# wafgo/rt-depth-map

Measured on AMD Instinct MI355X. Metric: stereo-pairs/sec, 1280x720 d=64 9x9 SAD, higher is better.
Workload: dtype u8

## Files before the change

rt-depth-map_amd/csrc/k_search_ring.hip:

```cpp
#include "rtdm_select.h"
#include "rtdm_border.h"
#include "rtdm_border2.h"

#include <cmath>
#include <cstdlib>
#include <type_traits>
#include <utility>

#ifndef RING_ABL
#define RING_ABL 0
#endif
#ifndef RING_LDS_SELECT
#define RING_LDS_SELECT 1
#endif
#ifndef RING_MINREC
#define RING_MINREC 1
#endif
#ifndef RING_W3_LIMIT
#define RING_W3_LIMIT 112
#endif
#ifndef RING_STATIC_SLOTS
#define RING_STATIC_SLOTS 1
#endif
#ifndef RING_DIRECT_LOADS
#define RING_DIRECT_LOADS 1
#endif
#ifndef RING_B64REC
#define RING_B64REC 1
#endif
#ifndef RING_MINREC96
#define RING_MINREC96 1
#endif
#ifndef RING_SPLIT_SELECT
#define RING_SPLIT_SELECT 0
#endif

#ifdef RING_STAMPS
__device__ unsigned long long ring_stamps[8];
#define RING_STAMP(i) do { unsigned long long t_; asm volatile("s_memtime %0\n\ts_waitcnt lgkmcnt(0)" : "=s"(t_) :: "memory"); \
                           stamp_sum[i] += t_ - stamp_last; stamp_last = t_; } while (0)
extern "C" void rtdm_debug_ring_stamps(unsigned long long* out, int reset)
{
    (void)hipMemcpyFromSymbol(out, HIP_SYMBOL(ring_stamps), sizeof(unsigned long long) * 8);
    if (reset) { unsigned long long z[8] = {0}; (void)hipMemcpyToSymbol(HIP_SYMBOL(ring_stamps), z, sizeof z); }
}
#else
#define RING_STAMP(i) do { } while (0)
#endif

namespace rtdm {

struct RingGeom {
    int x0, nx;
    int rs;
    uint32_t lastmask;
    int tiles, strips;
    unsigned nitems;
    unsigned chunk;
    uint32_t rdelta;
    int rebase;
    unsigned nborder;
    int bgx, bgy;
    int b2;
};

#ifndef RING_RPG96
#define RING_RPG96 4
#endif
#ifndef RING_RPG128
#define RING_RPG128 4
#endif
#ifndef RING_RPG256
#define RING_RPG256 4
#endif
__host__ __device__ constexpr int ring_rpg(int D, int LPP)
{ return D == 256 ? RING_RPG256 : D >= 192 ? 4 : D == 128 ? RING_RPG128 : D == 96 ? RING_RPG96 : LPP; }

template <int D, int WS, int LPP = 2>
struct RingCfg {
    static constexpr int RPG = ring_rpg(D, LPP);
    static constexpr bool SPLIT = LPP != 2 || D >= 48 || (D == 32 && (WS == 9 || WS == 5)) || (RING_SPLIT_SELECT && RING_LDS_SELECT);
    static constexpr bool MINREC = SPLIT && RING_MINREC && !(D == 128 && RPG == 8) && !(D == 96 && !RING_MINREC96);
    static_assert(RPG == LPP || MINREC, "GroupSelect's lane reductions need one owner per lane of a pixel");
    static constexpr bool B64 = MINREC && D == 64 && RING_B64REC;
    using Rec = SelRecord<D, MINREC || !SPLIT, B64>;
    static constexpr int NP = (WS + 3) / 4;
    static constexpr int W1 = WS + 1;
    static constexpr int PPW = 64 / LPP;
    static constexpr int DL = D / LPP;
    static constexpr int NGL = DL / 4;
    static constexpr int NRL = DL / 2;
    static constexpr int NW = NGL + NP - 1;
    static constexpr int LWD = PPW + NP;
    static constexpr int RWD = PPW + D / 4 + NP;
    static constexpr int ITEMS = (LWD + RWD + 63) / 64;
    static constexpr int SLOT = ITEMS * 64;
    static constexpr int TRIP = (W1 % RPG == 0) ? W1 : (2 * W1 % RPG == 0) ? 2 * W1 : 4 * W1;
    static_assert(W1 % 2 == 0 && TRIP % RPG == 0 && TRIP % W1 == 0, "block sizes are odd");
    static constexpr bool STATIC_SLOTS = RING_STATIC_SLOTS && ITEMS == 1 && TRIP % 4 == 0;
    static constexpr int NSLOT = STATIC_SLOTS ? 4 : 3;
    static constexpr int STG = (NSLOT * SLOT + (W1 + RPG) * PPW / 2 + 3) & ~3;
    static constexpr int WAVE_LDS = STG + PPW * RPG * Rec::DWORDS;
    static constexpr int RING_REGS = W1 * NRL;
    static constexpr int WAVES = LPP >= 8 ? 2 : LPP == 4 ? (RING_REGS <= (MINREC ? 80 : 64) ? 4 : (RING_REGS <= 96 && NRL <= 8) ? 3 : 2) : (RING_REGS <= 72 && NRL <= 8) ? 4 : RING_REGS <= RING_W3_LIMIT ? 3 : 2;
    static constexpr int TILE = 4 * PPW;
    static constexpr bool FUSE_BORDER = WAVES < 4;
    static constexpr bool FUSE_BORDER2 = D <= 192;
    static constexpr bool ROW_PTRS = !(LPP == 2 && RING_REGS > 88 && WAVES == 3);
};

template <int D, int WS, int LPP, bool BORDER>
#ifndef RING_BORDER_RELAX
#define RING_BORDER_RELAX 1
#endif
struct RingBounds { static constexpr int WAVES = RING_BORDER_RELAX && BORDER && RingCfg<D, WS, LPP>::WAVES > 1 ? RingCfg<D, WS, LPP>::WAVES - 1 : RingCfg<D, WS, LPP>::WAVES; };

template <int D, int WS, int LPP = 2>
struct RingState { uint64_t P[RingCfg<D, WS, LPP>::W1][RingCfg<D, WS, LPP>::NGL]; };

template <int D, int WS, int LPP = 2>
struct RowRegs { uint64_t win[RingCfg<D, WS, LPP>::NW]; uint32_t l[RingCfg<D, WS, LPP>::NP]; };

typedef __attribute__((address_space(3))) const uint32_t* lds_cptr;
__device__ __forceinline__ uint32_t lds_addr(const uint32_t* q) { return (uint32_t)(uintptr_t)(lds_cptr)q; }
__device__ __forceinline__ lds_cptr lds_at(uint32_t a) { return (lds_cptr)(uintptr_t)a; }

template <int D, int WS, int LPP, typename PTR>
__device__ __forceinline__ void ring_load_row(PTR lp, PTR rp, PTR rpo, RowRegs<D, WS, LPP>& rw)
{
    using C = RingCfg<D, WS, LPP>;
#pragma unroll
    for (int k = 0; k < C::NP; ++k) rw.l[k] = lp[k];
#pragma unroll
    for (int j = 0; j < C::NW; ++j) {
        const PTR wp = (j & 1) ? rpo + (j - 1) : rp + j;
        rw.win[j] = (uint64_t)wp[0] | ((uint64_t)wp[1] << 32);
    }
}

template <int D, int WS, int LPP, int K, int NRLc>
__device__ __forceinline__ void ring_step(RingState<D, WS, LPP>& st, const RowRegs<D, WS, LPP>& rw, uint32_t lastmask, uint32_t capb,
                                          uint32_t& tnew, uint32_t (&S)[NRLc])
{
    using C = RingCfg<D, WS, LPP>;
    auto& P = st.P;
    constexpr int NP = C::NP, NGL = C::NGL, W1 = C::W1;
    constexpr int KP = (K + W1 - 1) % W1, KO = (K + 1) % W1;
    uint32_t l[NP];
#pragma unroll
    for (int k = 0; k < NP; ++k) l[k] = rw.l[k];
    l[NP - 1] &= lastmask;
#pragma unroll
    for (int k = 0; k < NP - 1; ++k) tnew = __builtin_amdgcn_sad_u8(l[k], capb, tnew);
    tnew = __builtin_amdgcn_msad_u8(capb, l[NP - 1], tnew);
#pragma unroll
    for (int j = 0; j < C::NW; ++j) {
#pragma unroll
        for (int k = 0; k < NP; ++k) {
            const int gi = j - k;
            if (gi >= 0 && gi < NGL) {
                const uint64_t acc = k == 0 ? P[KP][gi] : P[K][gi];
#if RING_ABL == 4
                P[K][gi] = acc + (rw.win[j] ^ l[k]);
#else
                if (k == NP - 1) P[K][gi] = __builtin_amdgcn_mqsad_pk_u16_u8(rw.win[j], l[k], acc);
                else             P[K][gi] = __builtin_amdgcn_qsad_pk_u16_u8(rw.win[j], l[k], acc);
#endif
            }
        }
    }
#pragma unroll
    for (int gi = 0; gi < NGL; ++gi) {
        S[2 * gi] = (uint32_t)P[K][gi] - (uint32_t)P[KO][gi];
        S[2 * gi + 1] = (uint32_t)(P[K][gi] >> 32) - (uint32_t)(P[KO][gi] >> 32);
    }
}

template <int N>
__device__ __forceinline__ void pin(uint32_t (&v)[N])
{
#pragma unroll
    for (int i = 0; i < N; ++i) asm volatile("" : "+v"(v[i]));
}

template <typename F, int... U>
__device__ __forceinline__ void ring_for_groups(std::integer_sequence<int, U...>, F&& f)
{ (void)(f(std::integral_constant<int, U>{}) && ...); }
template <typename F, int... R>
__device__ __forceinline__ void ring_for_rows(std::integer_sequence<int, R...>, F&& f)
{ (f(std::integral_constant<int, R>{}), ...); }

template <int D, int WS, int LPP, bool FUSE>
__global__ __launch_bounds__(256, (RingBounds<D, WS, LPP, FUSE>::WAVES)) void k_search_ring(Plane8 Lp, Plane8 Rp, Plane16W disp, uint16_t* cost, BMGeom g, RingGeom rg,
                                                                                   BorderGeom bg, Border2Geom b2g)
{
    using C = RingCfg<D, WS, LPP>;
    constexpr int NGL = C::NGL, NRL = C::NRL, W1 = C::W1, LWD = C::LWD, SLOT = C::SLOT, ITEMS = C::ITEMS, PPW = C::PPW, RPG = C::RPG;
    constexpr bool SPLIT = C::SPLIT, MINREC = C::MINREC;
    constexpr int RECD = C::Rec::DWORDS;
    extern __shared__ __attribute__((aligned(16))) uint32_t lds[];

    unsigned fi = blockIdx.x;
    if constexpr (FUSE) {
        if (fi < rg.nborder) {
            const unsigned per = (unsigned)(rg.bgx * rg.bgy), fr = fi / per, id = fi - fr * per;
            if (C::FUSE_BORDER2 && rg.b2) {
                const int wave = __builtin_amdgcn_readfirstlane((int)(threadIdx.x >> 6));
                border2_body<D, C::NP>(Lp, Rp, disp, cost, g, b2g, (int)(id % rg.bgx) * 4 + wave, (int)(id / rg.bgx), (int)fr);
            } else if constexpr (C::FUSE_BORDER) {
                border_body<(D + 63) / 64>((unsigned char*)lds, Lp, Rp, disp, cost, g, bg, (int)(id % rg.bgx), (int)(id / rg.bgx), (int)fr);
            }
            return;
        }
        fi -= rg.nborder;
    }
    if (rg.chunk) fi = (fi & 7u) * rg.chunk + (fi >> 3);
    if (fi >= rg.nitems) return;
    const int b_tile = (int)(fi % rg.tiles), b_strip = (int)((fi / rg.tiles) % rg.strips), f = (int)(fi / (rg.tiles * rg.strips));

    const int tid = threadIdx.x, lane = tid & 63;
    const int phi = __builtin_amdgcn_readfirstlane(tid >> 6);
    const int p = lane & (PPW - 1), h = lane / PPW;
    const int x_tile = rg.x0 + b_tile * C::TILE;
    const int x = x_tile + phi + 4 * p;
    const bool active = x < rg.x0 + rg.nx;
    const int ys0 = g.vy0 + b_strip * rg.rs;
    const int ys1 = min(ys0 + rg.rs, g.vy1);
    if (ys0 >= ys1) return;
    const int r = g.r;
    const uint8_t* Lb = Lp.base + (size_t)f * Lp.frame;
#if !RING_DIRECT_LOADS
    const uint8_t* Rb = Rp.base + (size_t)f * Rp.frame;
#endif
    const int Lbase = g.lofs + x_tile - r + phi;
    const int Rbase = g.rofs + x_tile - r + phi;
    const uint32_t capb = (uint32_t)(g.cap + PREFILTER_BIAS) * 0x01010101u;

    uint32_t* stg = lds + phi * C::WAVE_LDS;
    unsigned short* ptr = (unsigned short*)(stg + C::NSLOT * SLOT);
    unsigned short* ptw = ptr + W1 * PPW;
    const bool owner = RPG == LPP || h < RPG;
    const unsigned short* ptw_own = ptw + (owner ? h : 0) * PPW + p;
    uint32_t* scr = stg + C::STG + (owner ? lane : 0) * RECD;
    uint32_t* scr_w = stg + C::STG + p * RECD + h * NRL;
    using GSel = std::conditional_t<MINREC, GroupSelectRec<D, LPP, C::B64>, GroupSelect<D, LPP>>;
    unsigned short* scr_m = (unsigned short*)(stg + C::STG + p * RECD + D / 2) + h * (NRL / 4);
    if constexpr (MINREC) GSel::init(scr);

    const int row0 = ys0 - r;
    const int Hm1 = g.H - 1;
#if RING_DIRECT_LOADS
    const uint8_t* rowp = Lb + (size_t)row0 * Lp.pitch;
    uint32_t loff[ITEMS];
#pragma unroll
    for (int it = 0; it < ITEMS; ++it) {
        const int idx = lane + it * 64;
        const bool isr = idx >= LWD;
        const int m = isr ? idx - LWD : idx;
        loff[it] = (uint32_t)((isr ? Rbase : Lbase) + 4 * m) + (isr ? rg.rdelta : 0u);
    }
    int next_row = row0;
    uint32_t pre[2][ITEMS];
    auto issue = [&](auto Sc) {
        constexpr int SET = decltype(Sc)::value;
#pragma unroll
        for (int it = 0; it < ITEMS; ++it) {
#if RING_ABL == 3
            pre[SET][it] = (uint32_t)next_row * 0x01020304u + lane;
#else
            asm volatile("" : "+v"(loff[it]));
            pre[SET][it] = *(const uint32_t*)(rowp + loff[it]);
#endif
        }
        rowp += next_row < Hm1 ? Lp.pitch : 0;
        ++next_row;
    };
    auto commit = [&](auto Sc, auto slot) {
        constexpr int SET = decltype(Sc)::value;
#pragma unroll
        for (int it = 0; it < ITEMS; ++it) stg[slot * SLOT + lane + it * 64] = pre[SET][it];
        __builtin_amdgcn_wave_barrier();
    };
#else
    const uint8_t* src[ITEMS];
    int it_sh[ITEMS];
#pragma unroll
    for (int it = 0; it < ITEMS; ++it) {
        const int idx = lane + it * 64;
        const bool isr = idx >= LWD;
        const int m = isr ? idx - LWD : idx;
        const int col = (isr ? Rbase : Lbase) + 4 * m;
        src[it] = (isr ? Rb : Lb) + (size_t)row0 * Lp.pitch + (col & ~3);
        it_sh[it] = col & 3;
    }
    int next_row = row0;
    uint32_t pre[2][ITEMS][2];
    auto issue = [&](auto Sc) {
        constexpr int SET = decltype(Sc)::value;
#pragma unroll
        for (int it = 0; it < ITEMS; ++it) {
#if RING_ABL == 3
            pre[SET][it][0] = (uint32_t)next_row * 0x01020304u + lane; pre[SET][it][1] = (uint32_t)next_row * 0x04030201u ^ lane;
#else
            pre[SET][it][0] = *(const uint32_t*)(src[it]);
            pre[SET][it][1] = *(const uint32_t*)(src[it] + 4);
#endif
        }
        const size_t adv = next_row < Hm1 ? Lp.pitch : 0;
#pragma unroll
        for (int it = 0; it < ITEMS; ++it) src[it] += adv;
        ++next_row;
    };
    auto commit = [&](auto Sc, auto slot) {
        constexpr int SET = decltype(Sc)::value;
#pragma unroll
        for (int it = 0; it < ITEMS; ++it) {
            const uint32_t v = __builtin_amdgcn_alignbyte(pre[SET][it][1], pre[SET][it][0], (uint32_t)it_sh[it]);
            stg[slot * SLOT + lane + it * 64] = v;
        }
        __builtin_amdgcn_wave_barrier();
    };
#endif
    using Set0 = std::integral_constant<int, 0>;
    using Set1 = std::integral_constant<int, 1>;

    RingState<D, WS, LPP> st;
#pragma unroll
    for (int k = 0; k < W1; ++k)
#pragma unroll
        for (int i = 0; i < NGL; ++i) st.P[k][i] = 0;
#pragma unroll
    for (int k = 0; k < W1; ++k) ptr[k * PPW + p] = 0;
    uint32_t pt = 0;

    const int nsteps = (ys1 - ys0) + WS - 1;
    const int nstepsg = (nsteps + RPG - 1) / RPG * RPG;
    issue(Set0{}); issue(Set1{});
    commit(Set0{}, 0); commit(Set1{}, 1);
    issue(Set0{});

    char* const db = (char*)(disp.base + (size_t)f * disp.frame_e);
    char* const cb = (char*)(cost + (size_t)f * g.H * g.Ws);
    const int col = g.lofs + x;
    constexpr int TF = (WS - 1) / RPG * RPG;
    uint32_t dofs = (uint32_t)(((long long)(ys0 + TF + h - (WS - 1)) * (long long)disp.pitch_e + col) * 2);
    uint32_t cofs = (uint32_t)(((long long)(ys0 + TF + h - (WS - 1)) * (long long)g.Ws + col) * 2);
    const uint32_t dstep = (uint32_t)(disp.pitch_e * 2 * RPG), cstep = (uint32_t)(g.Ws * 2 * RPG);
    const bool masked_col = g.mask_cols && (col < g.vx0 || col >= g.vx1);

    uint32_t S[RPG][NRL];
#ifdef RING_STAMPS
    unsigned long long stamp_sum[8] = {0, 0, 0, 0, 0, 0, 0, 0}, stamp_last;
    asm volatile("s_memtime %0\n\ts_waitcnt lgkmcnt(0)" : "=s"(stamp_last) :: "memory");
#endif
    int sl_cur = 0;
    uint32_t la_cur = lds_addr(stg + p), ra_cur = lds_addr(stg + LWD + p + h * NGL), ro_cur = ra_cur + 4;
    if constexpr (C::STATIC_SLOTS) asm volatile("" : "+v"(la_cur), "+v"(ra_cur), "+v"(ro_cur));
    const auto lds_row = [&](auto SLc, RowRegs<D, WS, LPP>& rw) {
        if constexpr (C::STATIC_SLOTS) {
            constexpr uint32_t off = (uint32_t)(decltype(SLc)::value * SLOT * 4);
            ring_load_row<D, WS, LPP>(lds_at(la_cur + off), lds_at(ra_cur + off), lds_at(ro_cur + off), rw);
        } else if constexpr (C::ROW_PTRS) {
            asm volatile("" : "+v"(la_cur), "+v"(ra_cur), "+v"(ro_cur));
            ring_load_row<D, WS, LPP>(lds_at(la_cur), lds_at(ra_cur), lds_at(ro_cur), rw);
            const uint32_t adv = (uint32_t)((sl_cur == 2 ? -2 * SLOT : SLOT) * 4);
            la_cur += adv; ra_cur += adv; ro_cur += adv;
        } else {
            int li = sl_cur * SLOT + p, ri = sl_cur * SLOT + LWD + p + h * NGL, one = 1;
            asm volatile("" : "+v"(li), "+v"(ri), "+v"(one));
            ring_load_row<D, WS, LPP, const uint32_t*>(stg + li, stg + ri, stg + ri + one, rw);
        }
    };
    auto step = [&](auto Kc, auto SLc, auto Rc, const RowRegs<D, WS, LPP>& rw, uint32_t (&Sr)[NRL]) {
        constexpr int K = decltype(Kc)::value;
        using SetIn = std::integral_constant<int, (K + 1) & 1>;
        using SetOut = std::integral_constant<int, K & 1>;
        issue(SetIn{});
        uint32_t tnew = 0;
        ring_step<D, WS, LPP, K>(st, rw, rg.lastmask, capb, tnew, Sr);
        constexpr int KO = (K + 1) % W1;
        pt += tnew;
        const uint32_t told = ptr[KO * PPW + p];
        ptr[K * PPW + p] = (unsigned short)pt;
        ptw[decltype(Rc)::value * PPW + p] = (unsigned short)(pt - told);
        pin(Sr);
        if constexpr (C::STATIC_SLOTS) {
            commit(SetOut{}, std::integral_constant<int, (decltype(SLc)::value + 2) % 4>{});
        } else {
            const int sl_new = sl_cur == 0 ? 2 : sl_cur - 1;
            sl_cur = sl_cur == 2 ? 0 : sl_cur + 1;
            commit(SetOut{}, sl_new);
        }
    };

    int trips_since_rebase = 0;
    for (int t0 = 0; t0 < nstepsg; t0 += C::TRIP) {
        if (rg.rebase && ++trips_since_rebase > rg.rebase) {
            trips_since_rebase = 1;
#pragma unroll
            for (int i = 0; i < NGL; ++i) {
                const uint32_t blo = (uint32_t)st.P[1][i], bhi = (uint32_t)(st.P[1][i] >> 32);
#pragma unroll
                for (int k = 1; k < W1; ++k) {
                    const uint32_t lo = (uint32_t)st.P[k][i] - blo, hi = (uint32_t)(st.P[k][i] >> 32) - bhi;
                    st.P[k][i] = (uint64_t)lo | ((uint64_t)hi << 32);
                }
            }
        }
        ring_for_groups(std::make_integer_sequence<int, C::TRIP / RPG>{}, [&](auto Uc) -> bool {
            constexpr int U = RPG * decltype(Uc)::value;
            const int t = t0 + U;
            if (t >= nstepsg) return false;
            RING_STAMP(0);
            GSel gsel;
            ring_for_rows(std::make_integer_sequence<int, RPG>{}, [&](auto Rc) {
                constexpr int R = decltype(Rc)::value;
                RowRegs<D, WS, LPP> rw;
                using SL = std::integral_constant<int, (U + R) % 4>;
                lds_row(SL{}, rw);
                RING_STAMP(1);
                step(std::integral_constant<int, (U + R) % W1>{}, SL{}, Rc, rw, S[R]);
                RING_STAMP(2);
                if constexpr (SPLIT && RING_ABL == 0) {
                    if constexpr (MINREC) gsel.template row<R>(S[R], scr_w + R * (PPW * RECD), scr_m + R * (PPW * RECD * 2));
                    else gsel.template row<R>(S[R], scr_w + R * (PPW * RECD), (uint32_t)(h * (NRL / 4)));
                }
            });
            if (t + RPG - 1 < WS - 1) return true;
            const int y = ys0 + (t - (WS - 1)) + h;
            const bool row_ok = owner && y >= ys0 && y < ys1;
            const uint32_t dof = dofs, cof = cofs;
            dofs += dstep; cofs += cstep;
            const int tsum = *ptw_own;
            const bool dead = !active | !row_ok | masked_col | (tsum < g.tex);
            if (__builtin_amdgcn_ballot_w64(!dead) == 0) {
                if (active && row_ok) *(int16_t*)(db + dof) = (int16_t)g.filtered;
            } else {
                int m1; bool fail;
                int out;
                if constexpr (SPLIT && MINREC && RING_ABL == 0) {
                    int uq = g.uniq;
                    asm volatile("" : "+s"(uq));
                    out = gsel.finish(tsum, g, uq > 0, scr, &m1, &fail);
                    RING_STAMP(5);
                } else if constexpr (SPLIT && RING_ABL == 0) {
                    out = gsel.finish(tsum, g, scr, &m1, &fail);
                    RING_STAMP(5);
                } else {
                    uint32_t rr[D / 2];
#pragma unroll
                    for (int i = 0; i < NRL; ++i) {
#if RING_ABL == 5 || RING_ABL == 6
                        rr[i] = S[0][i]; rr[NRL + i] = S[RPG - 1][i];
#else
                        const auto sw = __builtin_amdgcn_permlane32_swap(S[0][i], S[RPG - 1][i], false, false);
                        rr[i] = sw[0]; rr[NRL + i] = sw[1];
#endif
                    }
                    RING_STAMP(5);
#if RING_ABL == 1 || RING_ABL == 6
                    uint32_t xo = 0;
#pragma unroll
                    for (int i = 0; i < D / 2; ++i) xo ^= rr[i];
                    out = (int)xo; m1 = (int)(xo >> 3); fail = (xo & 1) != 0;
#elif RING_LDS_SELECT
                    out = select_disparity_lds<D>(rr, tsum, g, scr, &m1, &fail);
#else
                    out = select_disparity<D>(rr, tsum, g, &m1, &fail);
#endif
                }
#if RING_ABL == 2
                if (active && row_ok && out == 0x12345678) {
#else
                if (active && row_ok) {
#endif
                    if (!fail && g.want_cost) *(uint16_t*)(cb + cof) = (uint16_t)m1;
                    *(int16_t*)(db + dof) = (int16_t)(masked_col ? g.filtered : out);
                }
            }
            RING_STAMP(6);
            return true;
        });
    }
#ifdef RING_STAMPS
    if (lane == 0) for (int i = 0; i < 8; ++i) atomicAdd(&ring_stamps[i], stamp_sum[i]);
#endif
}

static bool ring_range(const BMGeom& g, int* x0, int* nx)
{
    const int r = g.r;
    int xl = 0, xh = g.width1 - 1;
    xl = max(xl, r - g.lofs); xl = max(xl, r - g.rofs);
    xh = min(xh, g.W - 1 - g.lofs - r); xh = min(xh, g.W - g.D - g.rofs - r);
    xl = max(xl, g.cx0 - g.lofs); xh = min(xh, g.cx1 - g.lofs - 1);
    if (x0) *x0 = xl;
    if (nx) *nx = xh - xl + 1;
    return xh >= xl;
}

static int ring_rows_cap(const BMGeom& g) { return 65535 / (g.w * 2 * g.cap) - g.w - 6; }
static int ring_lpp(const BMGeom& g);
static int ring_rebase_trips(const BMGeom& g)
{
    const int lpp = ring_lpp(g);
    if (!lpp) return 0;
    const int W1 = g.w + 1, rpg = ring_rpg(g.D, lpp);
    const int trip = (W1 % rpg == 0) ? W1 : (2 * W1 % rpg == 0) ? 2 * W1 : 4 * W1;
    return ring_rows_cap(g) / trip;
}
static int ring_min_strips(const BMGeom& g, int nrows)
{ return ring_rebase_trips(g) > 0 ? 1 : max(1, (nrows + ring_rows_cap(g) - 1) / ring_rows_cap(g)); }

#ifdef RTDM_RING_DEV
#define RTDM_RING_TABLE(X) RTDM_RING_DEV
#else
#define RTDM_RING_TABLE(X) X(64, 9, 2) X(64, 7, 2) X(64, 5, 2) X(32, 7, 2) X(32, 9, 2) X(32, 11, 2) X(32, 13, 2) X(48, 7, 2) X(48, 9, 2) \
                           X(16, 5, 2) X(16, 7, 2) X(16, 9, 2) X(64, 9, 4) X(64, 7, 4) X(64, 5, 4) X(64, 11, 4) X(64, 13, 4) \
                           X(128, 7, 8) X(128, 9, 8) X(128, 11, 8) X(128, 13, 8) X(96, 7, 4) X(96, 9, 4) X(96, 11, 4) X(96, 13, 4) X(48, 11, 2) X(48, 13, 2) \
                           X(16, 11, 2) X(16, 13, 2) X(32, 5, 2) X(32, 15, 2) X(48, 5, 2) X(64, 15, 4) X(128, 15, 8) \
                           X(192, 9, 8) X(192, 11, 8) X(192, 13, 8) X(192, 15, 8) X(256, 9, 16) X(256, 11, 16) X(256, 13, 16) X(256, 15, 16)
#endif

static std::atomic<int> g_ring_switch{0};
void ring_set_mode(int mode)
{
    const int m = mode < 0 ? -1 : mode == 0 ? 0 : 1, lpp = (mode == 2 || mode == 4 || mode == 8) ? mode : 0;
    g_ring_switch.store((m + 1) | (lpp << 8), std::memory_order_relaxed);
}
static int ring_mode() { return (g_ring_switch.load(std::memory_order_relaxed) & 0xff) - 1; }
static int ring_forced_lpp() { return g_ring_switch.load(std::memory_order_relaxed) >> 8; }

static int ring_lpp(const BMGeom& g)
{
    int have = 0;
#define X(DD, WW, LL) if (g.D == DD && g.w == WW) have |= LL;
    RTDM_RING_TABLE(X)
#undef X
    const int want = ring_forced_lpp();
    if (want && (have & want) == want) return want;
    return (have & 16) ? 16 : (have & 8) ? 8 : (have & 4) ? 4 : (have & 2) ? 2 : 0;
}

int ring_lanes_per_pixel(const BMGeom& g) { return ring_lpp(g); }

static int ring_tile(const BMGeom& g) { return 256 / ring_lpp(g); }

static int ring_wgs_per_cu(const BMGeom& g)
{
    const int lpp = ring_lpp(g);
#define X(DD, WW, LL) if (g.D == DD && g.w == WW && lpp == LL) return RingCfg<DD, WW, LL>::WAVES;
    RTDM_RING_TABLE(X)
#undef X
    return 2;
}

int ring_strips_model(const BMGeom& g, int n)
{
    int x0 = 0, nx = 0;
    if (!ring_range(g, &x0, &nx) || !ring_lpp(g)) return 1;
    const int tile = ring_tile(g), tiles = (nx + tile - 1) / tile, nrows = g.vy1 - g.vy0;
    const int slots = 256 * ring_wgs_per_cu(g);
    const int smin = ring_min_strips(g, nrows), smax = max(smin, (nrows + 15) / 16);
    const float fill = 0.5f * (float)(g.w - 1);
    int s = (int)(sqrtf((float)nrows * (float)slots / (fill * (float)tiles * (float)n)) + 0.5f);
    s = max(smin, min(s, smax));
    if ((long)tiles * s * n < 6L * slots) {
        float best = 1e30f;
        for (int c = smin; c <= smax; ++c) {
            const int rs = (nrows + c - 1) / c, ce = (nrows + rs - 1) / rs;
            const long rounds = ((long)tiles * ce * n + slots - 1) / slots;
            const float t = (float)rounds * ((float)rs + fill + 2.0f);
            if (t < best) { best = t; s = ce; }
        }
    }
    return s;
}

template <int D, int WS, int LPP>
static bool ring_launch_one(Plane8 Lp, Plane8 Rp, Plane16W disp, void* cost, const BMGeom& g, int n, hipStream_t stream, int strips_hint,
                            bool fuse_border)
{
    using C = RingCfg<D, WS, LPP>;
    RingGeom rg;
    rg.rdelta = (uint32_t)(Rp.base - Lp.base);
    ring_range(g, &rg.x0, &rg.nx);
    const int rem = g.w - 4 * (C::NP - 1);
    rg.lastmask = rem >= 4 ? 0xffffffffu : ((1u << (8 * rem)) - 1u);
    const int nrows = g.vy1 - g.vy0;
    const int tiles = (rg.nx + C::TILE - 1) / C::TILE;
    int strips = strips_hint > 0 ? strips_hint : ring_strips_model(g, n);
    strips = max(strips, ring_min_strips(g, nrows));
    rg.rebase = ring_rebase_trips(g);
    strips = max(1, min(strips, nrows));
    rg.rs = (nrows + strips - 1) / strips;
    strips = (nrows + rg.rs - 1) / rg.rs;
    rg.tiles = tiles; rg.strips = strips;
    rg.nitems = (unsigned)tiles * strips * n;
    rg.chunk = (rg.nitems + 7) / 8;
    const unsigned grid = rg.chunk * 8;
    BorderGeom bg{};
    Border2Geom b2g{};
    size_t blds = 0;
    rg.nborder = 0; rg.bgx = rg.bgy = 0; rg.b2 = 0;
    bool fused = false;
    if (fuse_border) {
        int lx0, lx1, rx0, rx1;
        fast_border_ranges(g, &lx0, &lx1, &rx0, &rx1);
        if (C::FUSE_BORDER2 && border2_plan(g, lx0, lx1, rx0, rx1, &b2g, &rg.bgx, &rg.bgy)) {
            rg.b2 = 1; fused = true;
            rg.nborder = (unsigned)(rg.bgx * rg.bgy) * (unsigned)n;
        } else if constexpr (C::FUSE_BORDER) {
            if (border_geometry(g, lx0, lx1, rx0, rx1, n, &bg, &rg.bgx, &rg.bgy, &blds)) { rg.nborder = (unsigned)(rg.bgx * rg.bgy) * (unsigned)n; fused = true; }
        }
    }
    const size_t ldsb = max((size_t)4 * C::WAVE_LDS * sizeof(uint32_t), blds);
    const auto launch = [&](auto Fc) {
        constexpr bool F = decltype(Fc)::value;
        constexpr size_t ring_lds = (size_t)4 * C::WAVE_LDS * sizeof(uint32_t);
        const size_t most = C::FUSE_BORDER ? max(ring_lds, border_lds_bytes(D, WS)) : ring_lds;
        static OncePerDevice once;
        if (most > 48 * 1024 && once.first()) {
            int dev = 0, lds_max = 0;
            size_t want = max(most, (size_t)64 * 1024);
            if (hipGetDevice(&dev) == hipSuccess &&
                hipDeviceGetAttribute(&lds_max, hipDeviceAttributeMaxSharedMemoryPerMultiprocessor, dev) == hipSuccess && lds_max > 0)
                want = min(want, (size_t)lds_max);
            (void)hipGetLastError();
            (void)hipFuncSetAttribute((const void*)k_search_ring<D, WS, LPP, F>, hipFuncAttributeMaxDynamicSharedMemorySize, (int)want);
        }
        hipLaunchKernelGGL((k_search_ring<D, WS, LPP, F>), dim3(grid + rg.nborder), dim3(256), ldsb, stream, Lp, Rp, disp, (uint16_t*)cost, g, rg, bg, b2g);
    };
    if (rg.nborder) { launch(std::true_type{}); return true; }
    launch(std::false_type{});
    return fused;
}

bool ring_search_supported(const BMGeom& g)
{
    if (ring_mode() == 0) return false;
    if (2L * g.cap * g.w * g.w > 32766) return false;
    if (2L * g.cap * g.w * g.w >= 0x7C00) return false;
    if (ring_rows_cap(g) < 2) return false;
    if (!ring_range(g, nullptr, nullptr)) return false;
    if ((size_t)g.H * (size_t)g.Ws * 2 >= ((size_t)1 << 32)) return false;
    return ring_lpp(g) != 0;
}

bool launch_search_ring(Plane8 Lp, Plane8 Rp, Plane16W disp, void* cost, const BMGeom& g, int n, hipStream_t stream, int strips_hint,
                        bool fuse_border)
{
    const int lpp = ring_lpp(g);
    if (RING_DIRECT_LOADS && !(Rp.base > Lp.base && (size_t)(Rp.base - Lp.base) < ((size_t)1 << 32) - ((size_t)1 << 20) && Rp.pitch == Lp.pitch && Rp.frame == Lp.frame)) {
        launch_search_fast(Lp, Rp, disp, cost, g, n, stream, fuse_border, 0);
        return fuse_border;
    }
#define X(DD, WW, LL) if (g.D == DD && g.w == WW && lpp == LL) return ring_launch_one<DD, WW, LL>(Lp, Rp, disp, cost, g, n, stream, strips_hint, fuse_border);
    RTDM_RING_TABLE(X)
#undef X
    return false;
}

}
```

Measured before the change: 73100.

## Distribute texture SAD per row-group lane instead of every lane computing it

When four rows share a group (TEX_OWN), each lane computes the texture prefilter SAD for only the one row it owns, loading that row from its own LDS slot. It then combines the four per-row terms with udot2 weights to form a running prefix sum in a per-pixel LDS ring, replacing the redundant per-row texture SAD and prefix bookkeeping done by every lane in ring_step. This reduces duplicated VALU SAD work and LDS writes per step. In exchange it adds extra LDS loads and stores, memory fences and a changed LDS layout for the texture ring.

```diff
diff --git a/rt-depth-map_amd/csrc/k_search_ring.hip b/rt-depth-map_amd/csrc/k_search_ring.hip
--- a/rt-depth-map_amd/csrc/k_search_ring.hip
+++ b/rt-depth-map_amd/csrc/k_search_ring.hip
@@ -99,7 +99,11 @@
     static_assert(W1 % 2 == 0 && TRIP % RPG == 0 && TRIP % W1 == 0, "block sizes are odd");
     static constexpr bool STATIC_SLOTS = RING_STATIC_SLOTS && ITEMS == 1 && TRIP % 4 == 0;
     static constexpr int NSLOT = STATIC_SLOTS ? 4 : 3;
-    static constexpr int STG = (NSLOT * SLOT + (W1 + RPG) * PPW / 2 + 3) & ~3;
+    static constexpr bool TEX_OWN = STATIC_SLOTS && RPG == 4 && WS >= RPG;
+    static constexpr int tex_slots() { int n = RPG; while (n < WS || TRIP % n) n += RPG; return n; }
+    static constexpr int NTR = tex_slots();
+    static constexpr int TBLK = NTR + 2 * RPG;
+    static constexpr int STG = (NSLOT * SLOT + (TEX_OWN ? PPW * TBLK : (W1 + RPG) * PPW) / 2 + 3) & ~3;
     static constexpr int WAVE_LDS = STG + PPW * RPG * Rec::DWORDS;
     static constexpr int RING_REGS = W1 * NRL;
     static constexpr int WAVES = LPP >= 8 ? 2 : LPP == 4 ? (RING_REGS <= (MINREC ? 80 : 64) ? 4 : (RING_REGS <= 96 && NRL <= 8) ? 3 : 2) : (RING_REGS <= 72 && NRL <= 8) ? 4 : RING_REGS <= RING_W3_LIMIT ? 3 : 2;
@@ -138,6 +142,14 @@
     }
 }
 
+template <int NP>
+__device__ __forceinline__ uint32_t ring_tex(const uint32_t (&l)[NP], uint32_t lastmask, uint32_t capb, uint32_t acc)
+{
+#pragma unroll
+    for (int k = 0; k < NP - 1; ++k) acc = __builtin_amdgcn_sad_u8(l[k], capb, acc);
+    return __builtin_amdgcn_msad_u8(capb, l[NP - 1] & lastmask, acc);
+}
+
 template <int D, int WS, int LPP, int K, int NRLc>
 __device__ __forceinline__ void ring_step(RingState<D, WS, LPP>& st, const RowRegs<D, WS, LPP>& rw, uint32_t lastmask, uint32_t capb,
                                           uint32_t& tnew, uint32_t (&S)[NRLc])
@@ -149,10 +161,8 @@
     uint32_t l[NP];
 #pragma unroll
     for (int k = 0; k < NP; ++k) l[k] = rw.l[k];
+    if constexpr (!C::TEX_OWN) tnew = ring_tex<NP>(l, lastmask, capb, tnew);
     l[NP - 1] &= lastmask;
-#pragma unroll
-    for (int k = 0; k < NP - 1; ++k) tnew = __builtin_amdgcn_sad_u8(l[k], capb, tnew);
-    tnew = __builtin_amdgcn_msad_u8(capb, l[NP - 1], tnew);
 #pragma unroll
     for (int j = 0; j < C::NW; ++j) {
 #pragma unroll
@@ -241,6 +251,9 @@
     unsigned short* ptw = ptr + W1 * PPW;
     const bool owner = RPG == LPP || h < RPG;
     const unsigned short* ptw_own = ptw + (owner ? h : 0) * PPW + p;
+    const int hr = h & (RPG - 1);
+    uint32_t tb_p = lds_addr((const uint32_t*)(ptr + p * C::TBLK)), tb_ph = tb_p + 2 * hr;
+    const uint32_t tw_lo = 1u | ((uint32_t)(hr >= 1) << 16), tw_hi = (uint32_t)(hr >= 2) | ((uint32_t)(hr >= 3) << 16);
     uint32_t* scr = stg + C::STG + (owner ? lane : 0) * RECD;
     uint32_t* scr_w = stg + C::STG + p * RECD + h * NRL;
     using GSel = std::conditional_t<MINREC, GroupSelectRec<D, LPP, C::B64>, GroupSelect<D, LPP>>;
@@ -329,8 +342,13 @@
     for (int k = 0; k < W1; ++k)
 #pragma unroll
         for (int i = 0; i < NGL; ++i) st.P[k][i] = 0;
-#pragma unroll
-    for (int k = 0; k < W1; ++k) ptr[k * PPW + p] = 0;
+    if constexpr (C::TEX_OWN) {
+#pragma unroll
+        for (int k = 0; k < (C::NTR + RPG) / RPG; ++k) ptr[p * C::TBLK + hr + k * RPG] = 0;
+    } else {
+#pragma unroll
+        for (int k = 0; k < W1; ++k) ptr[k * PPW + p] = 0;
+    }
     uint32_t pt = 0;
 
     const int nsteps = (ys1 - ys0) + WS - 1;
@@ -356,6 +374,8 @@
     int sl_cur = 0;
     uint32_t la_cur = lds_addr(stg + p), ra_cur = lds_addr(stg + LWD + p + h * NGL), ro_cur = ra_cur + 4;
     if constexpr (C::STATIC_SLOTS) asm volatile("" : "+v"(la_cur), "+v"(ra_cur), "+v"(ro_cur));
+    uint32_t la_own = la_cur + (uint32_t)(hr * SLOT * 4);
+    if constexpr (C::TEX_OWN) asm volatile("" : "+v"(la_own), "+v"(tb_p), "+v"(tb_ph));
     const auto lds_row = [&](auto SLc, RowRegs<D, WS, LPP>& rw) {
         if constexpr (C::STATIC_SLOTS) {
             constexpr uint32_t off = (uint32_t)(decltype(SLc)::value * SLOT * 4);
@@ -378,11 +398,13 @@
         issue(SetIn{});
         uint32_t tnew = 0;
         ring_step<D, WS, LPP, K>(st, rw, rg.lastmask, capb, tnew, Sr);
-        constexpr int KO = (K + 1) % W1;
-        pt += tnew;
-        const uint32_t told = ptr[KO * PPW + p];
-        ptr[K * PPW + p] = (unsigned short)pt;
-        ptw[decltype(Rc)::value * PPW + p] = (unsigned short)(pt - told);
+        if constexpr (!C::TEX_OWN) {
+            constexpr int KO = (K + 1) % W1;
+            pt += tnew;
+            const uint32_t told = ptr[KO * PPW + p];
+            ptr[K * PPW + p] = (unsigned short)pt;
+            ptw[decltype(Rc)::value * PPW + p] = (unsigned short)(pt - told);
+        }
         pin(Sr);
         if constexpr (C::STATIC_SLOTS) {
             commit(SetOut{}, std::integral_constant<int, (decltype(SLc)::value + 2) % 4>{});
@@ -413,25 +435,52 @@
             if (t >= nstepsg) return false;
             RING_STAMP(0);
             GSel gsel;
+            uint32_t tx = 0;
             ring_for_rows(std::make_integer_sequence<int, RPG>{}, [&](auto Rc) {
                 constexpr int R = decltype(Rc)::value;
                 RowRegs<D, WS, LPP> rw;
                 using SL = std::integral_constant<int, (U + R) % 4>;
+                uint32_t tl[C::NP];
+                if constexpr (C::TEX_OWN && R == 2) {
+                    const lds_cptr q = lds_at(la_own);
+#pragma unroll
+                    for (int k = 0; k < C::NP; ++k) tl[k] = q[k];
+                }
                 lds_row(SL{}, rw);
                 RING_STAMP(1);
                 step(std::integral_constant<int, (U + R) % W1>{}, SL{}, Rc, rw, S[R]);
+                if constexpr (C::TEX_OWN && R == 2) tx = ring_tex<C::NP>(tl, rg.lastmask, capb, 0u);
                 RING_STAMP(2);
                 if constexpr (SPLIT && RING_ABL == 0) {
                     if constexpr (MINREC) gsel.template row<R>(S[R], scr_w + R * (PPW * RECD), scr_m + R * (PPW * RECD * 2));
                     else gsel.template row<R>(S[R], scr_w + R * (PPW * RECD), (uint32_t)(h * (NRL / 4)));
                 }
             });
+            int tsum = 0;
+            if constexpr (C::TEX_OWN) {
+                constexpr int NTR = C::NTR, c = U % NTR;
+                typedef __attribute__((address_space(3))) unsigned short* lds_u16p;
+                typedef __attribute__((address_space(3))) const uint64_t* lds_u64cp;
+                asm volatile("" ::: "memory");
+                *(lds_u16p)(uintptr_t)(tb_ph + 2 * (NTR + RPG)) = (unsigned short)tx;
+                asm volatile("" ::: "memory");
+                const uint32_t base = ((lds_u16p)(uintptr_t)tb_p)[(c + NTR - 1) % NTR];
+                const uint32_t told = ((lds_u16p)(uintptr_t)tb_ph)[(c + NTR - WS) % NTR];
+                const uint64_t terms = *(lds_u64cp)(uintptr_t)(tb_p + 2 * (NTR + RPG));
+                asm volatile("" ::: "memory");
+                const uint32_t pre = __builtin_amdgcn_udot2(__builtin_bit_cast(sel_us2, (uint32_t)terms), __builtin_bit_cast(sel_us2, tw_lo),
+                                                            __builtin_amdgcn_udot2(__builtin_bit_cast(sel_us2, (uint32_t)(terms >> 32)),
+                                                                                   __builtin_bit_cast(sel_us2, tw_hi), base, false), false);
+                ((lds_u16p)(uintptr_t)tb_ph)[c] = (unsigned short)pre;
+                if constexpr (c == 0) ((lds_u16p)(uintptr_t)tb_ph)[NTR] = (unsigned short)pre;
+                tsum = (int)(unsigned short)(pre - told);
+            }
             if (t + RPG - 1 < WS - 1) return true;
             const int y = ys0 + (t - (WS - 1)) + h;
             const bool row_ok = owner && y >= ys0 && y < ys1;
             const uint32_t dof = dofs, cof = cofs;
             dofs += dstep; cofs += cstep;
-            const int tsum = *ptw_own;
+            if constexpr (!C::TEX_OWN) tsum = *ptw_own;
             const bool dead = !active | !row_ok | masked_col | (tsum < g.tex);
             if (__builtin_amdgcn_ballot_w64(!dead) == 0) {
                 if (active && row_ok) *(int16_t*)(db + dof) = (int16_t)g.filtered;
```

New measurement: 70430, median of 2. -3.6%, worse.
